# eBay/Sequence-Semantic-Embedding

Hardware: AMD Instinct MI355X
Metric: encoded seqs/sec (+ query x target cosine-scores/sec, top-1 vs ref) (higher is better)
Workload: dtype f32; 1 GPU; configs[1]: classification stand-in, dual-encoder LSTM H=S=256 E=50 T=32 V=32000; encode 16384 source seqs/GPU/step + cosine top-10 vs 571-target index; batch_per_gpu=16384, seq_len=32, targets=571, parallelism=dp1, weights=random-init (reference initialisers, seed 0)

## Files before the change

### sequence-semantic-embedding_amd/csrc/score_topk.hip

```cpp
#include <cstdlib>

#include "sse_kernels.h"
#include "score_exact.h"

#define SC_THREADS 512
#define SC_KC 16
#ifndef SC_PRIO_K
#define SC_PRIO_K 1
#define SC_PRIO_E 0
#endif

#ifdef SSE_SCORE_CLOCK
#include <cstdio>
__device__ long long g_score_clk[8 * 8];
#define SC_CLK_DECL long long ck_[8] = {0, 0, 0, 0, 0, 0, 0, 0}, ck_t = clock64();
#define SC_CLK(i)                   \
  {                                 \
    const long long n_ = clock64(); \
    ck_[i] += n_ - ck_t;            \
    ck_t = n_;                      \
  }
#else
#define SC_CLK_DECL
#define SC_CLK(i)
// ... 1093 lines not shown
bool score_small_index_applies(int Q, int KG, int64_t NT) {
  return Q >= 1024 && (KG == 32 || KG == 8 || KG == 7) && NT * 32 <= 1024 && (size_t)32 * (NT * 32 + 1) * sizeof(float) <= (size_t)144 * 1024;
}
hipError_t launch_score_small_index(const SmallIndexArgs &a, hipStream_t stream) {
  if (!score_small_index_applies(a.Q, a.KG, a.NT)) return hipErrorInvalidValue;
  const size_t lds = (size_t)32 * (a.NT * 32 + 1) * sizeof(float);
  const dim3 grid((a.Q + 31) / 32), block(256);
  auto go = [&](auto kernel) -> hipError_t {
    hipError_t e = hipFuncSetAttribute(reinterpret_cast<const void *>(kernel), hipFuncAttributeMaxDynamicSharedMemorySize, (int)lds);
    if (e != hipSuccess) return e;
    hipLaunchKernelGGL(kernel, grid, block, lds, stream, a);
    return hipGetLastError();
  };
  if (a.idx_x3 && a.KG != 32) return go(score_small_index_x3_kernel<4>);
  if (a.KG == 8) return go(score_small_index_kernel<8>);
  if (a.KG == 7) return go(score_small_index_kernel<7>);
  const hipError_t e32 = a.idx_x3 ? go(score_small_index_x3_kernel<16>) : go(score_small_index_kernel<32>);
  if (e32 != hipSuccess) return e32;
#ifdef SSE_SCORE_CLOCK
  if (a.Q >= 8192) {
    static int n = 0;
    if (n++ % 8 == 3) {
      long long v[64];
      (void)hipStreamSynchronize(stream);
      (void)hipMemcpyFromSymbol(v, HIP_SYMBOL(g_score_clk), sizeof v);
      for (int w = 0; w < 4; w += 3)
        fprintf(stderr, "[small index clock Q=%d NT=%d] wave %d cycles: query fragments %lld | scores (MFMA + LDS stores) %lld | barrier %lld | selection: loads + bounds %lld | bisection %lld | winners + rank + stores %lld (both batches)\n",
                a.Q, a.NT, w, v[w * 8 + 0], v[w * 8 + 1], v[w * 8 + 2], v[w * 8 + 5], v[w * 8 + 6], v[w * 8 + 3] + v[w * 8 + 4]);
    }
  }
#endif
  return hipGetLastError();
}

hipError_t launch_score_topk(const ScoreArgs &a_in, hipStream_t stream) {
  ScoreArgs a = a_in;
#ifdef SSE_SCORE_MEASURE
  {
    static const int dbg = getenv("SSE_SCORE_DBG") ? atoi(getenv("SSE_SCORE_DBG")) : 0;
    a.dbg = dbg;
  }
#endif
  if (a.KC != SC_KC) return hipErrorInvalidValue;
  if (a.q_rows && ((a.NQ != 1 && !a.COLLECT) || a.S < 1)) return hipErrorInvalidValue;
  if (a.NSPLIT > 8 && (a.NSPLIT & 7)) return hipErrorInvalidValue;
  if (a.NSPLIT < 8 && (8 % a.NSPLIT)) return hipErrorInvalidValue;
  if (a.COLLECT) {
    if (!a.lane_max && (!a.col_thr || !a.col_slot || !a.col_cnt || !a.col_buf)) return hipErrorInvalidValue;
    if (a.BF) return a.NQ == 4 ? launch_score_variant<4, true, true>(a, stream) : hipErrorInvalidValue;
    if (a.NQ == 1) return launch_score_variant<1, false, true>(a, stream);
    if (a.NQ == 2) return launch_score_variant<2, false, true>(a, stream);
    if (a.NQ == 4) return launch_score_variant<4, false, true>(a, stream);
    return hipErrorInvalidValue;
  }
  if (!a.part_bnd) return hipErrorInvalidValue;
  if (a.BF) {
    if (a.NQ == 1) return launch_score_variant<1, true, false>(a, stream);
    if (a.NQ == 2) return launch_score_variant<2, true, false>(a, stream);
    if (a.NQ == 4) return launch_score_variant<4, true, false>(a, stream);
    return hipErrorInvalidValue;
  }
  if (a.NQ == 1) return launch_score_variant<1, false, false>(a, stream);
  if (a.NQ == 2) return launch_score_variant<2, false, false>(a, stream);
  if (a.NQ == 4) return launch_score_variant<4, false, false>(a, stream);
  return hipErrorInvalidValue;
}


template <int NB>
__device__ __forceinline__ int packed_value_of_lane(int lane) {
  int v = 0;
#pragma unroll
  for (int cnt = NB, bit = 5; cnt > 1; cnt >>= 1, --bit) v = v * 2 + ((lane >> bit) & 1);
  return v;
}
template <int NB>
__device__ __forceinline__ int packed_lane_of_value(int v) {
  int lane = 0;
#pragma unroll
  for (int cnt = NB, bit = 5; cnt > 1; cnt >>= 1, --bit) lane |= ((v / (cnt / 2)) & 1) << bit;
  return lane;
}
template <int NB>
__device__ __forceinline__ double wave_exact_dot_packed(const float *qrow, const float *idxp, const double *idx64, const int64_t (&n)[NB],
                                                        int S, int KG, int lane, const float *idx_rm = nullptr) {
  static_assert(NB == 2 || NB == 4 || NB == 8, "power of two");
  double acc[NB];
#pragma unroll
  for (int b = 0; b < NB; ++b) acc[b] = 0.0;
  if (idx64) {
    for (int d = lane; d < S; d += 64) {
      double rv[NB];
#pragma unroll
      for (int b = 0; b < NB; ++b) rv[b] = idx64[(size_t)n[b] * S + d];
#pragma unroll
      for (int b = 0; b < NB; ++b) acc[b] += (double)qrow[d] * rv[b];
    }
  } else {
    for (int j = lane; j < KG * 2; j += 64) {
      const int kg = j >> 1, half = j & 1;
      f32x4 v[NB];
#pragma unroll
      for (int b = 0; b < NB; ++b)
        v[b] = idx_rm ? *reinterpret_cast<const f32x4 *>(idx_rm + (size_t)n[b] * S + j * 4)
                      : *reinterpret_cast<const f32x4 *>(idxp + (size_t)(n[b] >> 5) * KG * 256 + kg * 256 + (half * 32 + (int)(n[b] & 31)) * 4);
      const int d0 = kg * 8 + half * 4;
#pragma unroll
      for (int e = 0; e < 4; ++e)
        if (d0 + e < S) {
#pragma unroll
          for (int b = 0; b < NB; ++b) acc[b] += (double)qrow[d0 + e] * (double)v[b][e];
        }
    }
  }
  int m = 32;
#pragma unroll
  for (int cnt = NB; cnt > 1; cnt >>= 1, m >>= 1) {
    const bool up = (lane & m) != 0;
#pragma unroll
    for (int i = 0; i < cnt / 2; ++i) {
      const double send = up ? acc[i] : acc[i + cnt / 2];
      const double keep = up ? acc[i + cnt / 2] : acc[i];
      acc[i] = keep + __shfl_xor(send, m);
    }
  }
#pragma unroll
  for (; m > 0; m >>= 1) acc[0] += __shfl_xor(acc[0], m);
  return acc[0];
}

#define RS_THREADS 256
#define RS_MAXWIN 256
#define RS_MAXNC 4096
__global__ __launch_bounds__(RS_THREADS) void rescore_kernel(RescoreArgs a) {
  __shared__ int s_cnt;
  __shared__ int s_wid[RS_MAXWIN];
  __shared__ double s_ex[RS_MAXWIN];
  __shared__ float s_m[RS_THREADS / 64];
  __shared__ double s_qn[RS_THREADS / 64];
  extern __shared__ __attribute__((aligned(16))) unsigned long long s_key[];
  const int q = blockIdx.x, tid = threadIdx.x, lane = tid & 63, w = tid >> 6;
  if (a.uncert_clear && q == 0 && tid == 0) *a.uncert_clear = 0;
  if (a.q_count && q >= *a.q_count) return;
  const int qo = a.qmap ? a.qmap[q] : q;
  const float *ps = a.part_scores + (size_t)q * a.NC;
  const int32_t *pi = a.part_ids + (size_t)q * a.NC;
  const float *qrow = a.q + (size_t)q * a.S;
  const int KG = (a.S + 7) / 8;

  constexpr int PER = RS_MAXNC / RS_THREADS;
  float rs[PER];
  int ri[PER];
#pragma unroll
  for (int j = 0; j < PER; ++j) {
    const int c = tid + j * RS_THREADS;
    ri[j] = (c < a.NC) ? pi[c] : -1;
    rs[j] = (c < a.NC) ? ps[c] : NEG_INF;
  }
  float mmax = NEG_INF;
  for (int c = tid; c < a.NC / SC_KC; c += RS_THREADS) mmax = fmaxf(mmax, a.part_bnd[(size_t)q * (a.NC / SC_KC) + c]);

  {
    double v = 0.0;
    for (int d = tid; d < a.S; d += RS_THREADS) v += (double)qrow[d] * qrow[d];
#pragma unroll
    for (int o = 32; o > 0; o >>= 1) v += __shfl_xor(v, o);
    if (lane == 0) s_qn[w] = v;
  }
#pragma unroll
  for (int o = 32; o > 0; o >>= 1) mmax = fmaxf(mmax, __shfl_xor(mmax, o));
  if (lane == 0) s_m[w] = mmax;
  if (tid == 0) s_cnt = 0;

#pragma unroll
  for (int j = 0; j < PER; ++j) {
    const int c = tid + j * RS_THREADS;
    if (c < a.NC) {
      unsigned u = __float_as_uint(rs[j]);
      u = (u & 0x80000000u) ? ~u : (u | 0x80000000u);
      s_key[c] = (ri[j] < 0) ? 0ull : (((unsigned long long)u << 32) | (unsigned long long)(0xFFFFFFFFu - (unsigned)ri[j]));
    }
  }
  __syncthreads();
  const float qnorm = (float)sqrt(s_qn[0] + s_qn[1] + s_qn[2] + s_qn[3]);
  const float eps_q = a.eps * qnorm;
  mmax = fmaxf(fmaxf(s_m[0], s_m[1]), fmaxf(s_m[2], s_m[3]));
  float kth = NEG_INF;
  if (a.NC <= 256) {
    const unsigned long long key = (tid < a.NC) ? s_key[tid] : 0ull;
    int rank = 0;
    for (int j = 0; j < a.NC; ++j) rank += (s_key[j] > key) ? 1 : 0;
    float mine = (key != 0ull && rank == a.k - 1) ? rs[0] : NEG_INF;
#pragma unroll
    for (int o = 32; o > 0; o >>= 1) mine = fmaxf(mine, __shfl_xor(mine, o));
    __shared__ float s_thr[RS_THREADS / 64];
    if (lane == 0) s_thr[w] = mine;
    __syncthreads();
    kth = fmaxf(fmaxf(s_thr[0], s_thr[1]), fmaxf(s_thr[2], s_thr[3]));
  } else {
    __shared__ unsigned long long s_best[(RS_THREADS / 64) * SC_KC];
    const int nslots = a.NC / SC_KC;
    int head[RS_MAXNC / SC_KC / RS_THREADS];
#pragma unroll
    for (int j = 0; j < RS_MAXNC / SC_KC / RS_THREADS; ++j) head[j] = 0;
    for (int it = 0; it < a.k; ++it) {
      unsigned long long best = 0ull;
#pragma unroll
      for (int j = 0; j < RS_MAXNC / SC_KC / RS_THREADS; ++j) {
        const int slot = tid + j * RS_THREADS;
        if (slot < nslots && head[j] < SC_KC) {
          const unsigned long long key = s_key[slot * SC_KC + head[j]];
// ... 125 lines not shown
#endif
  const bool have = lane < a.NC;
  const int id = have ? a.part_ids[(size_t)q * a.NC + lane] : -1;
  const float sc = have ? a.part_scores[(size_t)q * a.NC + lane] : NEG_INF;
  const float bnd = (lane < a.NC / SC_KC) ? a.part_bnd[(size_t)q * (a.NC / SC_KC) + lane] : NEG_INF;
  double qn = 0.0;
  for (int d = lane; d < a.S; d += 64) qn += (double)qrow[d] * qrow[d];
#pragma unroll
  for (int o = 32; o > 0; o >>= 1) qn += __shfl_xor(qn, o);
  const float qnorm = (float)sqrt(qn);
  const float eps_q = a.eps * qnorm;
  RS_CLK(0)

  unsigned u = __float_as_uint(sc);
  u = (u & 0x80000000u) ? ~u : (u | 0x80000000u);
  const unsigned long long key = (id < 0) ? 0ull : (((unsigned long long)u << 32) | (unsigned long long)(0xFFFFFFFFu - (unsigned)id));
  const int key_lo = (int)(unsigned)key, key_hi = (int)(unsigned)(key >> 32);
  int rank = 0;
  for (int j = 0; j < a.NC; ++j) {
    const unsigned long long kj = ((unsigned long long)(unsigned)__builtin_amdgcn_readlane(key_hi, j) << 32) |
                                  (unsigned long long)(unsigned)__builtin_amdgcn_readlane(key_lo, j);
    rank += (kj > key) ? 1 : 0;
  }
  const unsigned long long kmask = __ballot(key != 0ull && rank == a.k - 1);
  const float kth = kmask ? __int_as_float(__builtin_amdgcn_readlane(__float_as_int(sc), __ffsll((long long)kmask) - 1)) : NEG_INF;
  const bool in_win = (id >= 0) && (sc >= kth - 2.0f * eps_q);
  float mmax = NEG_INF;
  for (int j = 0; j < a.NC / SC_KC; ++j) mmax = fmaxf(mmax, __int_as_float(__builtin_amdgcn_readlane(__float_as_int(bnd), j)));
  const unsigned long long wmask = __ballot(in_win);
  const int nwin = __popcll(wmask);
  const int mi = __popcll(wmask & ((1ull << lane) - 1ull));
  const int idm = __builtin_amdgcn_ds_permute((in_win ? mi : 63) * 4, id);
  RS_CLK(1)
  double exm = -__builtin_inf();
  for (int m0 = 0; m0 < nwin; m0 += RS_NB) {
    int64_t n[RS_NB];
#pragma unroll
    for (int c = 0; c < RS_NB; ++c) n[c] = __builtin_amdgcn_readlane(idm, (m0 + c < nwin) ? m0 + c : 0);
    const double tot = wave_exact_dot_packed<RS_NB>(qrow, a.idx32, a.idx64, n, a.S, KG, lane, a.idx_rm);
    const int want = lane - m0;
    const double got = __shfl(tot, packed_lane_of_value<RS_NB>(want & (RS_NB - 1)));
    if (want >= 0 && want < RS_NB && lane < nwin) exm = got;
  }
  RS_CLK(2)
  int r2 = 0;
  for (int j = 0; j < nwin; ++j)
    r2 += before(readlane_f64(exm, j), (int64_t)__builtin_amdgcn_readlane(idm, j), exm, (int64_t)idm) ? 1 : 0;
  const bool member = lane < nwin;
  if (member && r2 < a.k) {
    a.out_scores[(size_t)qo * a.k + r2] = exm;
    a.out_ids[(size_t)qo * a.k + r2] = a.id_base + idm;
    if (a.host_flag) {
      a.host_scores[(size_t)qo * a.k + r2] = exm;
      a.host_ids[(size_t)qo * a.k + r2] = a.id_base + idm;
    }
  }
  const unsigned long long tmask = __ballot(member && r2 == a.k - 1);
  const double theta = tmask ? readlane_f64(exm, __ffsll((long long)tmask) - 1) : -__builtin_inf();
  if (a.host_flag) __threadfence_system();
  RS_CLK(3)
#ifdef SSE_SCORE_CLOCK
  if (q == a.Q / 2 && lane == 0) {
    rk_[4] = nwin;
    for (int i = 0; i < 6; ++i) g_score_clk[i] = rk_[i];
  }
#endif
  if (lane == 0) {
    const bool ok = (nwin >= a.k) && ((double)mmax + (double)eps_q < theta);
    a.cert[qo] = ok ? 1 : 0;
    if (!ok && a.uncert) atomicAdd(a.uncert, 1);
    if (a.col_thr) a.col_thr[qo] = ok ? __builtin_inff() : __double2float_rd(theta - (double)(a.eps32 * qnorm));
    if (a.col_slot) {
      a.col_slot[qo] = ok ? -1 : qo;
      a.col_cnt[qo] = 0;
    }
    if (a.host_flag) {
      a.host_cert[qo] = ok ? 1 : 0;
      if (qo == 0 && a.host_err) *a.host_err = a.err_in ? *a.err_in : 0;
      __hip_atomic_store(a.host_flag + qo, a.seq, __ATOMIC_RELEASE, __HIP_MEMORY_SCOPE_SYSTEM);
    }
  }
}

hipError_t launch_rescore(const RescoreArgs &a, hipStream_t stream) {
  if (a.NC > RS_MAXNC) return hipErrorInvalidValue;
  if (a.NC <= 64) {
    hipLaunchKernelGGL(rescore_small_kernel, dim3((a.Q + 3) / 4), dim3(256), 0, stream, a);
#ifdef SSE_SCORE_CLOCK
    if (a.Q >= 8192) {
      static int n = 0;
      if (n++ % 8 == 3) {
        long long v[8];
        (void)hipStreamSynchronize(stream);
        (void)hipMemcpyFromSymbol(v, HIP_SYMBOL(g_score_clk), sizeof v);
        fprintf(stderr, "[rescore_small clock Q=%d NC=%d] cycles: query norm %lld | candidates, rank, k-th, window %lld | float64 dots %lld (window of %lld) | exact rank + outputs %lld\n",
                a.Q, a.NC, v[0], v[1], v[2], v[4], v[3]);
      }
    }
#endif
    return hipGetLastError();
  }
  hipLaunchKernelGGL(rescore_kernel, dim3(a.Q), dim3(RS_THREADS), (size_t)a.NC * sizeof(unsigned long long), stream, a);
  return hipGetLastError();
}

#define EX_THREADS 256
struct ExactArgs {
  const float *q;
  const float *idxp;
  const double *idx64;
  const int32_t *cert;
  double *out_scores;
  int64_t *out_ids;
  int64_t id_base, N;
  int32_t Q, S, k;
  int32_t k_off, k_total;
  unsigned long long *served;
  const int32_t *uncert;
};

__device__ __forceinline__ void exact_topk_query(const ExactArgs a, const int q, double (*s_sc)[SC_KC],
                                                 int64_t (*s_id)[SC_KC]) {
  const int tid = threadIdx.x, lane = tid & 63, w = tid >> 6;
  if (a.served && tid == 0 && a.k_off == 0) atomicAdd(a.served, 1ull);
  const float *qrow = a.q + (size_t)q * a.S;
  const int KG = (a.S + 7) / 8;
  double ls[SC_KC];
  int64_t li[SC_KC];
#pragma unroll
  for (int i = 0; i < SC_KC; ++i) {
    ls[i] = -__builtin_inf();
    li[i] = -1;
  }
  double cut_s = __builtin_inf();
  int64_t cut_id = -1;
  if (a.k_off > 0) {
    cut_s = a.out_scores[(size_t)q * a.k_total + a.k_off - 1];
    cut_id = a.out_ids[(size_t)q * a.k_total + a.k_off - 1] - a.id_base;
  }
  for (int64_t n = w; n < a.N; n += EX_THREADS / 64) {
    double s = wave_exact_dot(qrow, a.idxp, a.idx64, n, a.S, KG, lane);
    const bool after_cut = (s < cut_s) || (s == cut_s && n > cut_id);
    if (after_cut && s > ls[SC_KC - 1]) {
      int64_t id = n;
      bool ins = false;
#pragma unroll
      for (int i = 0; i < SC_KC; ++i) {
        const bool gt = ins || (s > ls[i]);
        ins = gt;
        const double tv = ls[i];
        const int64_t ti = li[i];
        ls[i] = gt ? s : tv;
        li[i] = gt ? id : ti;
        s = gt ? tv : s;
        id = gt ? ti : id;
      }
    }
  }
  if (lane == 0) {
#pragma unroll
    for (int i = 0; i < SC_KC; ++i) {
      s_sc[w][i] = ls[i];
      s_id[w][i] = li[i];
    }
  }
  __syncthreads();
  if (tid == 0) {
    unsigned pos4 = 0;
// ... 285 lines not shown
```

### sequence-semantic-embedding_amd/csrc/sse_api.hip

```cpp
#include <cmath>
#include <cstdarg>
#include <cstdio>
#include <cstdlib>
#include <algorithm>
#include <chrono>
#include <cstring>
#include <dlfcn.h>
#include <link.h>
#include <mutex>
#include <string>
#include <vector>

#include "../../include/sse_hip.h"
#include "sse_kernels.h"
#include "train.h"

namespace {

thread_local std::string g_create_error;

struct Variable {
  std::string name;
  int rows = 0, cols = 0;
  int64_t count = 0;
// ... 36 lines not shown
  size_t cap = 0;
  DevBuf() = default;
  DevBuf(const DevBuf &) = delete;
  DevBuf &operator=(const DevBuf &) = delete;
  ~DevBuf() {
    if (p) (void)hipFree(p);
  }
};

struct TrainState {
  DevBuf ids[2], labels, raw[2], draw[2], tape_g[2], tape_a[2], h_last[2], dh_last[2], dg_a[2], dg_b[2], db_part[2],
      dk_part[2], dm_part[2], sq_part, norm_part, row_loss, row_acc, scal;
  DevBuf feat_rm, pos, dfeat, dw_part, dbias_part, wt, wct;
  uint64_t gen_ver[2] = {0, 0};
  DevBuf gen_A[2], gen_tape[2], gen_dG[2], gen_hl[2], gen_KT[2], gen_Kq[2], gen_MT[2], gen_G, gen_c, gen_dA, gen_dc, gen_dkp;
  hipStream_t side[2] = {nullptr, nullptr};
  hipEvent_t ev_fork = nullptr, ev_join[2] = {nullptr, nullptr};
  float *KhT[2] = {nullptr, nullptr}, *KxT[2] = {nullptr, nullptr};
  unsigned short *KhT16[2] = {nullptr, nullptr};
  unsigned short *KxT16[2] = {nullptr, nullptr};
  bool packed_dirty = true;
  bool fp32_dirty = true;
  float *arena = nullptr;
  bool arena_external = false, grads_ready = false;
  DevBuf corpus[2], rows[2];
  int64_t corpus_N[2] = {0, 0};
  int32_t corpus_T[2] = {0, 0};
  bool rows_mode = false;
  bool defer_err = false;
  DevBuf ids_raw[2], perm, hot_part[2];
  int perm_B = 0;
  std::vector<int32_t> h_perm, h_rows[2], h_tgt;
  std::vector<float> h_labels;
};

}

enum { PATH_PERSIST, PATH_CLUSTER, PATH_SMALL, PATH_X3, PATH_GENERIC, PATH_FWD, PATH_FWD_ROWS32, PATH_FWD_ROWS64, PATH_FWD_GS, PATH_FWD_XT,
       PATH_COUNT };

struct sse_handle {
  sse_config cfg;
  std::mutex mu;
  std::string err;
  std::vector<Variable> vars;
  Encoder enc[2];
  bool packed_dirty = true;
  uint64_t weights_version = 1;
  bool mp_fresh = false;
  int pad_skip = 1;
  int pad_sort_dev = 1;
  int score_two_pass_min_rows = 49152, score_two_pass_rows = 524288;
  int64_t two_pass_calls = 0;
  DevBuf s_lmax;
  int lstm_gate_split = 1;
  DevBuf s_padzero, s_padwork, s_padorder;
  int32_t *pad_stat = nullptr;
  int32_t pad_seq = 0;
  int64_t pad_sorted_calls = 0;
  int64_t lstm_path_calls[PATH_COUNT] = {};
  int lstm_x3 = 0;
  unsigned short *emb16 = nullptr;
  bool emb16_valid = false;
  int lstm_persist_rows = 32;
  uint32_t persist_epoch = 0;
  hipStream_t stream = nullptr;
  int persist_inject = 0;
  int64_t persist_fallbacks = 0;
  int cu_count = 0;
  int lstm_cluster_rows = 1024;
  uint32_t cluster_epoch = 0;
  int lstm_cluster_chunks = 3;
  int cluster_backoff = -1;
  int cluster_skip[2] = {0, 0};
  int lstm_cluster_coop = 1;
  int lstm_cluster_wt = 0;
  int lstm_cluster_drop = 0;
  int lstm_small_rows = 1024;
  int lstm_x_table = 1;
  int lstm_x_table_mb = 256;
  int64_t x_table_builds = 0;
  int score_small_index = 1;
  int score_small_x3 = 1;
  int score_bf16 = 1;
  void *idxp16 = nullptr;
  size_t idxp16_cap = 0;
  bool idxp16_valid = false;
  bool fb_cnt_init = false;
  int uncert_word = 0;
  bool cnn_bf16 = false;
  unsigned short *emb_bf16 = nullptr, *cnn_Wc16 = nullptr, *cnn_Mx3 = nullptr;
  int lstm_train_rows = 0;
  int train_bwd_x3 = 0;
  int train_fwd_x3 = 0;
  int train_dk_x3 = 0;
  int train_generic = 0;
  int train_gen1 = 0;
  int train_pair_dedup = 1;
  int train_serial = 0;
  float *emb_pad = nullptr;
  int cnn_W[4] = {-1, -1, -1, -1}, cnn_b[4] = {-1, -1, -1, -1}, cnn_M = -1, tgt_table = -1;
  float *cnn_Wc = nullptr, *cnn_bias = nullptr, *cnn_Mp = nullptr;
  int32_t *err_flag = nullptr;
  float *idxp = nullptr;
  size_t idxp_cap = 0;
  double *idx64 = nullptr;
  DevBuf idx_rm;
  bool idx_rm_valid = false;
  DevBuf idx_x3;
  bool idx_x3_valid = false;
  int64_t idx_N = 0, idx_base = 0;
  int idx_S = 0;
  float idx_norm_max = 1.0f;
  DevBuf s_ids, s_out, s_q, s_qp, s_ps, s_pi, s_cert, s_os, s_oi, s_tmp, s_tmp2, s_feat, s_zero, s_map;
  DevBuf s_qmap, s_qc;
  DevBuf s_qp32, s_fb_cnt;
  DevBuf g_A, g_G, g_c, g_hl, g_raw;
  DevBuf g_KT[2], g_Kq[2], g_MT[2];
  uint64_t g_ver[2] = {0, 0};
  DevBuf s_xchg;
  DevBuf s_persist;
  DevBuf s_cluster;
  int32_t *pin_small = nullptr;
  void *pin = nullptr;
  size_t pin_cap = 0;
  int32_t score_seq = 0;
  DevBuf s_pb, s_cthr, s_cslot, s_ccnt, s_cbuf;
  DevBuf s_rk, s_rk_cnt;
  bool rk_cnt_init = false;
  DevBuf s_ab, s_ab_sort, s_ab_cnt, s_ab_out;
  bool ab_cnt_init = false;
  DevBuf idx_tags, idx_tag_sum, s_ft_max, s_ft_cnt;
  bool tags_set = false, ft_cnt_init = false;
  int score_filtered_skip = 1;
  DevBuf idx_groups, s_gp_max, s_gp_cnt;
  bool groups_set = false, gp_cnt_init = false;
  DevBuf s_af_bnd, s_af_cnt;
  bool af_cnt_init = false;
  DevBuf s_stage;
  int eval_chunk_rows = 65536;
  int64_t eval_paired_calls = 0;
  DevBuf ev_ids[2], ev_stage, ev_rows[2], ev_labels, ev_raw[2], ev_row, ev_sums;
  float lr = 0.9f;
  int64_t global_step = 0;
  TrainState *train = nullptr;
  std::vector<hipEvent_t> events;
};

namespace {

int fail(sse_handle *h, const char *fmt, ...) {
  char buf[512];
  va_list ap;
  va_start(ap, fmt);
  vsnprintf(buf, sizeof buf, fmt, ap);
  va_end(ap);
  if (h) h->err = buf; else g_create_error = buf;
  return 1;
}

#define HIPCHECK(h, expr)                                                                         \
  do {                                                                                            \
    hipError_t e_ = (expr);                                                                       \
    if (e_ != hipSuccess) return fail(h, "%s failed: %s (%s:%d)", #expr, hipGetErrorString(e_), __FILE__, __LINE__); \
  } while (0)

// ... 1345 lines not shown
    HIPCHECK(h, launch_exact_topk(q, h->idxp, h->idx64, (const int32_t *)h->s_cert.p, out_s, out_i, h->idx_base, h->idx_N, Q, S, k, st,
                                  counters + 2));
    if (split) *split = 0;
    return 0;
  }
  const int POOL = std::min(Q, 1024);
  if (reserve(h, h->s_qp, (size_t)QB * NQ * KG * 256 * sizeof(float))) return 1;
  if (reserve(h, h->s_ps, (size_t)Q * (bf ? NCmax : NC) * sizeof(float))) return 1;
  if (reserve(h, h->s_pi, (size_t)Q * (bf ? NCmax : NC) * sizeof(int32_t))) return 1;
  if (reserve(h, h->s_pb, (size_t)Q * (bf ? NCmax / 16 : nsplit) * sizeof(float))) return 1;
  if (reserve(h, h->s_cert, (size_t)Q * sizeof(int32_t))) return 1;
  if (reserve_collect(h, Q, POOL)) return 1;
  if (split) *split = 1;
  const bool first = phase != SCORE_REST, rest = phase != SCORE_FIRST;
  const bool rows_direct = NQ == 1;
  if (first && !rows_direct && !small_idx) {
    if (bf) HIPCHECK(h, launch_pack_rows_bf16(q, Q, S, h->s_qp.p, st));
    else HIPCHECK(h, launch_pack_rows(q, Q, S, (float *)h->s_qp.p, st));
  }
  ScoreArgs a;
  if (rows_direct) {
    a.q_rows = q;
    a.S = S;
  }
  a.BF = bf ? 1 : 0;
  a.idxp = bf ? (const float *)h->idxp16 : h->idxp;
  a.qp = (const float *)h->s_qp.p;
  a.part_scores = (float *)h->s_ps.p;
  a.part_ids = (int32_t *)h->s_pi.p;
  a.part_bnd = (float *)h->s_pb.p;
  a.N = h->idx_N;
  a.Q = Q;
  a.KG = bf ? KG16 : KG;
  a.NT = (int)NT;
  a.QT = QT;
  a.NSPLIT = nsplit;
  a.KC = 16;
  a.NQ = NQ;
  if (first) {
    if (small_idx) {
      SmallIndexArgs si{q, h->idxp, a.part_scores, a.part_ids, a.part_bnd, h->idx_N, Q, S, KG, (int)NT};
      if (small_x3) si.idx_x3 = h->idx_x3.p;
      HIPCHECK(h, launch_score_small_index(si, st));
    } else {
      HIPCHECK(h, launch_score_topk(a, st));
    }
  }
  RescoreArgs r;
  r.q = q;
  r.idx32 = h->idxp;
  r.idx64 = h->idx64;
  r.idx_rm = h->idx_rm_valid ? (const float *)h->idx_rm.p : nullptr;
  r.part_scores = a.part_scores;
  r.part_ids = a.part_ids;
  r.part_bnd = a.part_bnd;
  r.out_scores = out_s;
  r.out_ids = out_i;
  r.cert = (int32_t *)h->s_cert.p;
  r.id_base = h->idx_base;
  r.N = h->idx_N;
  r.Q = Q;
  r.S = S;
  r.NC = NC;
  r.k = k;
  const float eps32 = score_eps32(h);
  r.eps = eps32;
  r.eps32 = eps32;
  r.col_thr = (float *)h->s_cthr.p;
  if (first) h->uncert_word ^= 1;
  int32_t *const uncert = (int32_t *)(counters + 4) + h->uncert_word;
  const int follow_grid = 2 * (h->cu_count > 0 ? h->cu_count : 256);
  r.uncert = uncert;
  r.uncert_clear = (int32_t *)(counters + 4) + (h->uncert_word ^ 1);
  const bool own_slots = Q <= POOL;
  if (own_slots) {
    r.col_slot = (int32_t *)h->s_cslot.p;
    r.col_cnt = (int32_t *)h->s_ccnt.p;
  }
  if (bf) r.eps += (float)(1.02 * (1.0 / 256.0 + 1.0 / 262144.0) * h->idx_norm_max);
  if (small_x3)
    r.eps = (float)(((1.0 + 1.0 / 64.0) / 32768.0 + 2.0 * (3 * S + 2) * 5.97e-8 * (1.0 + 1.0 / 32.0)) * h->idx_norm_max);
  if (first) {
    RescoreArgs rf = r;
    if (mirror) {
      rf.host_scores = mirror->scores;
      rf.host_ids = mirror->ids;
      rf.host_cert = mirror->cert;
      rf.host_err = mirror->err;
      rf.host_flag = mirror->flag;
      rf.err_in = h->err_flag;
      rf.seq = mirror->seq;
    }
    HIPCHECK(h, launch_rescore(rf, st));
  }
  if (!rest) return 0;
  const float *qp32 = (const float *)h->s_qp.p;
  if (bf && Q > 32) {
    if (reserve(h, h->s_qp32, (size_t)QB * NQ * KG * 256 * sizeof(float))) return 1;
    if (reserve(h, h->s_qmap, (size_t)(Q + 1) * sizeof(int32_t))) return 1;
    if (reserve(h, h->s_qc, (size_t)QT * 32 * S * sizeof(float))) return 1;
    HIPCHECK(h, launch_count_uncert(r.cert, Q, counters, st));
    int32_t *qmap = (int32_t *)h->s_qmap.p, *qcount = qmap + Q;
    HIPCHECK(h, launch_compact_uncert(q, r.cert, Q, S, qmap, qcount, (float *)h->s_qc.p, st));
    if (!rows_direct) HIPCHECK(h, launch_pack_rows((const float *)h->s_qc.p, Q, S, (float *)h->s_qp32.p, st));
    ScoreArgs a2 = a;
    a2.BF = 0;
    a2.idxp = h->idxp;
    a2.qp = (const float *)h->s_qp32.p;
    if (rows_direct) a2.q_rows = (const float *)h->s_qc.p;
    a2.KG = KG;
    a2.q_count = qcount;
    a2.NSPLIT = nsplit2;
    HIPCHECK(h, launch_score_topk(a2, st));
    RescoreArgs r2 = r;
    r2.q = (const float *)h->s_qc.p;
    r2.NC = nsplit2 * 16;
    r2.eps = eps32;
    r2.qmap = qmap;
    r2.q_count = qcount;
    r2.uncert = r2.uncert_clear = nullptr;
    HIPCHECK(h, launch_rescore(r2, st));
    qp32 = (const float *)h->s_qp32.p;
  }
  if (!own_slots) {
    HIPCHECK(h, hipMemsetAsync(h->s_ccnt.p, 0, (size_t)(POOL + 1) * sizeof(int32_t), st));
    HIPCHECK(h, launch_assign_slots(r.cert, Q, POOL, (int32_t *)h->s_cslot.p, (int32_t *)h->s_ccnt.p + POOL, st));
  }
  ScoreArgs c = a;
  c.BF = 0;
  c.idxp = h->idxp;
  c.qp = qp32;
  c.q_rows = q;
  c.S = S;
  c.KG = KG;
  c.COLLECT = 1;
  c.col_thr = (const float *)h->s_cthr.p;
  c.col_slot = (const int32_t *)h->s_cslot.p;
  c.col_cnt = (int32_t *)h->s_ccnt.p;
  c.col_buf = (int32_t *)h->s_cbuf.p;
  c.col_cap = SSE_COLLECT_CAP;
  c.uncert = uncert;
  HIPCHECK(h, launch_score_topk(c, st));
  SelectArgs sel{q, h->idxp, h->idx64, c.col_slot, c.col_cnt, c.col_buf, SSE_COLLECT_CAP, out_s, out_i, r.cert, h->idx_base, Q, S, k,
                 counters + 1, uncert, follow_grid};
  HIPCHECK(h, launch_select_topk(sel, st));
  HIPCHECK(h, launch_exact_topk(q, h->idxp, h->idx64, r.cert, out_s, out_i, h->idx_base, h->idx_N, Q, S, k, st, counters + 2, uncert,
                                follow_grid));
  return 0;
}

}

extern "C" {

const char *sse_last_error(sse_handle *h) { return h ? h->err.c_str() : g_create_error.c_str(); }

int sse_create(const sse_config *cfg, sse_handle **out) {
  if (!cfg || !out) return fail(nullptr, "sse_create: null argument");
  *out = nullptr;
  int ndev = 0;
  if (hipGetDeviceCount(&ndev) != hipSuccess || ndev == 0) return fail(nullptr, "no HIP device available");
  if (cfg->device < 0 || cfg->device >= ndev) return fail(nullptr, "device %d out of range (have %d)", cfg->device, ndev);
  if (cfg->vocab_size < 2 || cfg->embedding_size < 1 || cfg->encoding_size < 1)
    return fail(nullptr, "bad model sizes V=%d E=%d S=%d", cfg->vocab_size, cfg->embedding_size, cfg->encoding_size);
  sse_handle *h = new sse_handle();
  h->cfg = *cfg;
// ... 349 lines not shown
  if (bits) {
    if (check_err_flag(h, nullptr, &bits)) return 1;
    if (bits == 4) {
      if (encode_fallback_locked(h, side, B, T, normalize, nullptr)) return 1;
      if (score_to_host_locked(h, (const float *)h->s_out.p, B, k, out_scores, out_ids)) return 1;
    }
  }
  if (enc_out_host)
    HIPCHECK(h, hipMemcpy(enc_out_host, h->s_out.p, (size_t)B * h->cfg.encoding_size * sizeof(float), hipMemcpyDeviceToHost));
  return 0;
}

namespace {

struct DevCounters {
  DevBuf sse_handle::*buf;
  bool sse_handle::*init;
  int words;
};
enum { CG_RANK, CG_ABOVE, CG_FILTERED, CG_GROUPED, CG_AFTER, CG_TOPK, CG_DEV_COUNT, CG_HOST = CG_DEV_COUNT, CG_PATH, CG_COOP };
const DevCounters DEV_COUNTERS[CG_DEV_COUNT] = {
    {&sse_handle::s_rk_cnt, &sse_handle::rk_cnt_init, 2}, {&sse_handle::s_ab_cnt, &sse_handle::ab_cnt_init, 3},
    {&sse_handle::s_ft_cnt, &sse_handle::ft_cnt_init, 3}, {&sse_handle::s_gp_cnt, &sse_handle::gp_cnt_init, 3},
    {&sse_handle::s_af_cnt, &sse_handle::af_cnt_init, 3}, {&sse_handle::s_fb_cnt, &sse_handle::fb_cnt_init, 4}};
int64_t sse_handle::*const HOST_COUNTERS[] = {&sse_handle::persist_fallbacks, &sse_handle::two_pass_calls, &sse_handle::pad_sorted_calls,
                                              &sse_handle::eval_paired_calls, &sse_handle::x_table_builds};

const struct {
  const char *name;
  int group, word;
} COUNTERS[] = {
    {"lstm_persist_fallbacks", CG_HOST, 0},
    {"score_two_pass_calls", CG_HOST, 1},
    {"pad_sorted_calls", CG_HOST, 2},
    {"eval_paired_calls", CG_HOST, 3},
    {"lstm_x_table_builds", CG_HOST, 4},
    {"lstm_path_persist", CG_PATH, PATH_PERSIST},
    {"lstm_path_cluster", CG_PATH, PATH_CLUSTER},
    {"lstm_path_small", CG_PATH, PATH_SMALL},
    {"lstm_path_x3", CG_PATH, PATH_X3},
    {"lstm_path_generic", CG_PATH, PATH_GENERIC},
    {"lstm_path_fwd", CG_PATH, PATH_FWD},
    {"lstm_fwd_rows32", CG_PATH, PATH_FWD_ROWS32},
    {"lstm_fwd_rows64", CG_PATH, PATH_FWD_ROWS64},
    {"lstm_fwd_gate_split", CG_PATH, PATH_FWD_GS},
    {"lstm_fwd_x_table", CG_PATH, PATH_FWD_XT},
    {"lstm_coop_refused", CG_COOP, 0},
    {"score_rank_band_rows", CG_RANK, 0},
    {"score_rank_bruteforce_pairs", CG_RANK, 1},
    {"score_above_band_rows", CG_ABOVE, 0},
    {"score_above_bruteforce_pairs", CG_ABOVE, 1},
    {"score_above_long_segments", CG_ABOVE, 2},
    {"score_filtered_collected_rows", CG_FILTERED, 0},
    {"score_filtered_bruteforce_queries", CG_FILTERED, 1},
    {"score_filtered_tiles_skipped", CG_FILTERED, 2},
    {"score_grouped_collected_rows", CG_GROUPED, 0},
    {"score_grouped_bruteforce_queries", CG_GROUPED, 1},
    {"score_after_collected_rows", CG_AFTER, 0},
    {"score_after_bruteforce_queries", CG_AFTER, 1},
    {"score_bf16_second_chance_queries", CG_TOPK, 0},
    {"score_collect_queries", CG_TOPK, 1},
    {"score_bruteforce_queries", CG_TOPK, 2},
};

static int read_dev_counter(sse_handle *h, const DevCounters &g, int word, int64_t *value) {
  unsigned long long v[4] = {0, 0, 0, 0};
  if ((h->*g.buf).p && h->*g.init) {
    HIPCHECK(h, hipSetDevice(h->cfg.device));
    HIPCHECK(h, hipDeviceSynchronize());
    HIPCHECK(h, hipMemcpy(v, (h->*g.buf).p, g.words * sizeof v[0], hipMemcpyDeviceToHost));
  }
  *value = (int64_t)v[word];
  return 0;
}

const struct {
  const char *name;
  int sse_handle::*member;
  int min, max;
  const char *message;
} OPTIONS[] = {
    {"score_small_index", &sse_handle::score_small_index},
    {"score_small_x3", &sse_handle::score_small_x3},
    {"score_filtered_skip", &sse_handle::score_filtered_skip},
    {"score_bf16", &sse_handle::score_bf16},
    {"train_bwd_x3", &sse_handle::train_bwd_x3},
    {"train_fwd_x3", &sse_handle::train_fwd_x3},
    {"train_dk_x3", &sse_handle::train_dk_x3},
    {"train_generic", &sse_handle::train_generic},
    {"train_gen1", &sse_handle::train_gen1},
    {"train_pair_dedup", &sse_handle::train_pair_dedup},
    {"train_serial", &sse_handle::train_serial},
    {"pad_skip", &sse_handle::pad_skip},
    {"lstm_gate_split", &sse_handle::lstm_gate_split},
    {"lstm_x3", &sse_handle::lstm_x3},
    {"lstm_persist_inject_miss", &sse_handle::persist_inject},
    {"lstm_cluster_drop_wg", &sse_handle::lstm_cluster_drop},
    {"lstm_cluster_coop", &sse_handle::lstm_cluster_coop},
    {"lstm_cluster_write_through", &sse_handle::lstm_cluster_wt},
    {"score_two_pass_min_rows", &sse_handle::score_two_pass_min_rows, 0, INT32_MAX, "score_two_pass_min_rows must be >= 0"},
    {"score_two_pass_rows", &sse_handle::score_two_pass_rows, 0, INT32_MAX, "score_two_pass_rows must be >= 0"},
    {"pad_sort_dev", &sse_handle::pad_sort_dev, 0, 2, "pad_sort_dev must be 0 (off), 1 (adaptive) or 2 (always)"},
    {"lstm_persist_rows", &sse_handle::lstm_persist_rows, 0, INT32_MAX, "lstm_persist_rows must be >= 0"},
    {"lstm_cluster_chunks", &sse_handle::lstm_cluster_chunks, 1, INT32_MAX, "lstm_cluster_chunks must be >= 1"},
    {"lstm_cluster_rows", &sse_handle::lstm_cluster_rows, 0, INT32_MAX, "lstm_cluster_rows must be >= 0"},
    {"lstm_small_rows", &sse_handle::lstm_small_rows, 0, INT32_MAX, "lstm_small_rows must be >= 0"},
    {"lstm_x_table", &sse_handle::lstm_x_table, 0, 2, "lstm_x_table must be 0 (off), 1 (batches with B * T >= vocab_size) or 2 (always)"},
    {"lstm_x_table_mb", &sse_handle::lstm_x_table_mb, 0, INT32_MAX, "lstm_x_table_mb must be >= 0"},
};

}

int sse_get_counter(sse_handle *h, const char *name, int64_t *value) {
  if (!h || !name || !value) return 1;
  std::lock_guard<std::mutex> lk(h->mu);
  for (const auto &c : COUNTERS) {
    if (strcmp(name, c.name) != 0) continue;
    if (c.group < CG_DEV_COUNT) return read_dev_counter(h, DEV_COUNTERS[c.group], c.word, value);
    *value = c.group == CG_HOST ? h->*HOST_COUNTERS[c.word] : c.group == CG_PATH ? h->lstm_path_calls[c.word] : (int64_t)lstm_coop_refused();
    return 0;
  }
  return fail(h, "unknown counter '%s'", name);
}

int sse_set_option(sse_handle *h, const char *name, int32_t value) {
  if (!h || !name) return 1;
  std::lock_guard<std::mutex> lk(h->mu);
  for (const auto &o : OPTIONS) {
    if (strcmp(name, o.name) != 0) continue;
    if (o.message && (value < o.min || value > o.max)) return fail(h, "%s", o.message);
    h->*o.member = o.message ? value : value != 0;
    return 0;
  }
  if (strcmp(name, "cnn_bf16") == 0) {
    if (h->cfg.network_mode != SSE_MODE_SOURCE_ONLY_CNN) return fail(h, "option cnn_bf16 needs network_mode source_only_cnn");
    h->cnn_bf16 = value != 0;
    h->packed_dirty = true;
    h->mp_fresh = false;
    return 0;
  }
  if (strcmp(name, "lstm_train_rows") == 0) {
    if (value != 0 && value != 32 && value != 64) return fail(h, "lstm_train_rows must be 0, 32 or 64");
    h->lstm_train_rows = (int)value;
    return 0;
  }
  if (strcmp(name, "eval_chunk_rows") == 0) {
    if (value < 2) return fail(h, "eval_chunk_rows must be >= 2");
    h->eval_chunk_rows = (int)(value & ~1);
    return 0;
  }
  if (strcmp(name, "lstm_persist_epoch") == 0) {
    if (value < 0 || value >= (1 << 20)) return fail(h, "lstm_persist_epoch must be in [0, 2^20)");
    h->persist_epoch = (uint32_t)value;
    return 0;
  }
  if (strcmp(name, "lstm_cluster_backoff") == 0) {
    if (value < -1) return fail(h, "lstm_cluster_backoff must be >= 0 (or -1: automatic)");
    h->cluster_backoff = (int)value;
    h->cluster_skip[0] = h->cluster_skip[1] = 0;
    return 0;
  }
  return fail(h, "unknown option '%s'", name);
}

int sse_l2_normalize_dev(sse_handle *h, const float *x_dev, float *out_dev, int64_t rows, int32_t cols, void *stream) {
  SSE_ENTER(h);
// ... 1279 lines not shown
```

### sequence-semantic-embedding_amd/csrc/sse_kernels.h

```cpp
#pragma once
#include <hip/hip_runtime.h>
#include <stdint.h>

typedef float f32x4 __attribute__((ext_vector_type(4)));
typedef float f32x16 __attribute__((ext_vector_type(16)));

__host__ __device__ static inline int frag32_off(int r_in_tile, int k_in_group) {
  return ((((k_in_group >> 2) << 5) + r_in_tile) << 2) + (k_in_group & 3);
}

__device__ static inline int mfma_row(int reg, int lane) { return (reg & 3) + 8 * (reg >> 2) + 4 * (lane >> 5); }

static inline int round_up(int x, int m) { return (x + m - 1) / m * m; }

typedef unsigned int sse_u32x4 __attribute__((ext_vector_type(4)));
__host__ __device__ static inline unsigned short sse_bf16_rne(float f) {
  unsigned u;
  __builtin_memcpy(&u, &f, 4);
  u += 0x7FFFu + ((u >> 16) & 1u);
  return (unsigned short)(u >> 16);
}
__host__ __device__ static inline float sse_bf16_f32(unsigned short h) {
  const unsigned u = (unsigned)h << 16;
  float f;
// ... 175 lines not shown
  int32_t B, T, V, E, Ep, KGx, KGh, H, Hp, S, NTS, normalize;
  const float *pad_h = nullptr, *pad_c = nullptr;
  int32_t pad_stride = 0;
  unsigned long long *hx = nullptr;
  unsigned long long *sx = nullptr;
  uint32_t epoch = 0;
  int32_t NCL = 0;
  int32_t write_through = 0;
  int32_t plain_launch = 0;
  int32_t drop_wg = 0;
};
int lstm_cluster_ok(int E, int H, int S);
int lstm_cluster_max_rows();
size_t lstm_cluster_weight_floats(int E, int H);
size_t lstm_cluster_hx_words(int H);
size_t lstm_cluster_sx_words();
hipError_t launch_pack_lstm_cluster(const float *K, const float *b, int E, int H, float *Wc, hipStream_t stream);
hipError_t launch_lstm_cluster(const LstmClusterArgs &a, hipStream_t stream);

struct ScoreArgs {
  const float *idxp;
  const float *qp;
  float *part_scores;
  int32_t *part_ids;
  float *part_bnd;
  int64_t N;
  int32_t Q, KG, NT, QT, NSPLIT, KC;
  int32_t NQ = 4;
  int32_t thr_off = 0;
  const int32_t *q_count = nullptr;
  int32_t BF = 0;
  int32_t COLLECT = 0;
  const float *col_thr = nullptr;
  const int32_t *col_slot = nullptr;
  int32_t *col_cnt = nullptr;
  int32_t *col_buf = nullptr;
  int32_t col_cap = 0;
  float *lane_max = nullptr;
  int32_t dbg = 0;
  const float *q_rows = nullptr;
  int32_t S = 0;
  const int32_t *uncert = nullptr;
};
hipError_t launch_score_topk(const ScoreArgs &a, hipStream_t stream);
hipError_t launch_lane_max_threshold(const float *q, const float *lane_max, int Q, int S, int NV, float eps, float *col_thr,
                                     int32_t *col_slot, hipStream_t st);
#define SSE_MAX_INDEX_DIM 1024
int score_pick_nq(int Q, int S, int with_bf16);
size_t score_lds_bytes(int NQ, int KG, int BF, int COLLECT);
hipError_t launch_pack_rows_bf16(const float *rows, int64_t R, int C, void *out, hipStream_t stream);
hipError_t launch_count_uncert(const int32_t *cert, int Q, unsigned long long *count, hipStream_t st);
hipError_t launch_compact_uncert(const float *q, const int32_t *cert, int Q, int S, int32_t *qmap, int32_t *count, float *qc,
                                 hipStream_t st);
hipError_t launch_frag32_to_bf16(const float *idxp, int64_t NT, int KG, void *out, hipStream_t stream);
hipError_t launch_frag32_to_split_bf16(const float *idxp, int64_t NT, int KG, void *out, hipStream_t stream);

#define SSE_COLLECT_CAP 4096
#define SSE_MAX_SELECT_K 1024

struct RescoreArgs {
  const float *q;
  const float *idx32;
  const double *idx64;
  const float *part_scores;
  const int32_t *part_ids;
  const float *part_bnd;
  double *out_scores;
  int64_t *out_ids;
  int32_t *cert;
  int64_t id_base, N;
  int32_t Q, S, NC, k;
  float eps;
  const int32_t *qmap = nullptr, *q_count = nullptr;
  float *col_thr = nullptr;
  float eps32 = 0.0f;
  int32_t *col_slot = nullptr, *col_cnt = nullptr;
  double *host_scores = nullptr;
  int64_t *host_ids = nullptr;
  int32_t *host_cert = nullptr, *host_flag = nullptr, *host_err = nullptr;
  const int32_t *err_in = nullptr;
  int32_t seq = 0;
  const float *idx_rm = nullptr;
  int32_t *uncert = nullptr, *uncert_clear = nullptr;
};
hipError_t launch_rescore(const RescoreArgs &a, hipStream_t stream);

struct SmallIndexArgs {
  const float *q_rows;
  const float *idxp;
  float *part_scores;
  int32_t *part_ids;
  float *part_bnd;
  int64_t N;
  int32_t Q, S, KG, NT;
  const void *idx_x3 = nullptr;
};
bool score_small_index_applies(int Q, int KG, int64_t NT);
hipError_t launch_score_small_index(const SmallIndexArgs &a, hipStream_t stream);

struct RankArgs {
  const float *q;
  const int32_t *pair_q;
  const int64_t *pair_id;
  const double *pair_score_in;
  const float *idxp;
  const double *idx64;
  int64_t *out_before;
  double *out_score;
  double *thr64;
  float *lo, *hi;
  unsigned long long *sure;
  int32_t *band_cnt, *band_buf;
  int32_t band_cap;
  const int32_t *bad;
  unsigned long long *counters;
  int64_t id_base, N;
  int32_t S, KG, NT, P, NSPLIT, NQ;
  float eps32;
};
hipError_t launch_rank_validate(const int32_t *pair_q, const int64_t *pair_id, int64_t L, int Q, int need_row, int64_t id_base,
                                int64_t N, int32_t *bad, int32_t *err_flag, hipStream_t st);
hipError_t launch_score_rank(const RankArgs &a, hipStream_t st);

struct AboveArgs {
  const float *q;
  const int32_t *pair_q;
  const double *pair_thr;
  const float *idxp;
  const double *idx64;
  float *lo, *hi;
  unsigned long long *sure;
  int32_t *band_cnt, *band_buf;
  int32_t band_cap;
  const int32_t *bad;
  int32_t *err_flag;
  unsigned long long *counters;
  int64_t *counts;
  const int64_t *offsets;
  const int64_t *total;
  int32_t *ovf;
  unsigned long long *cursor;
  int64_t *out_ids;
  int64_t cap;
  int64_t id_base, N;
  int32_t S, KG, NT, P, NSPLIT, NQ, emit;
  float eps32;
};
#define SSE_ABOVE_SORT_CAP 8192
hipError_t launch_above_validate(const int32_t *pair_q, int64_t L, int Q, int32_t *bad, int32_t *err_flag, hipStream_t st);
hipError_t launch_score_above(const AboveArgs &a, hipStream_t st);
hipError_t launch_above_scan(int64_t *offsets, int64_t L, const int32_t *bad, hipStream_t st);
struct AboveListArgs {
  const float *q;
  const int32_t *pair_q;
  const float *idxp;
  const double *idx64;
  const int64_t *offsets;
  const unsigned long long *cursor;
  int64_t *ids;
  double *scores;
  int64_t *scratch_ids;
  double *scratch_scores;
  const int32_t *bad;
  int32_t *err_flag;
  unsigned long long *counters;
  int64_t L, cap, id_base, N;
// ... 129 lines not shown
```

Before: 7.578 million seqs/s.

## Add row-packed rescore kernel handling four queries per wavefront with DPP ranking

Adds a specialised rescore kernel for 16-candidate partial results. Each 16-lane row of a wavefront handles one query, so four queries share a wave. Candidates are ranked with DPP row rotations instead of shared-memory sorting, and ranking is skipped when the small-index path already sorted them. Exact float64 dots are batched across the combined windows of all four queries, with double-buffered row loads. It is gated on NC==16, no qmap or host mirroring, and Q>=256, with an option flag to turn it off. The aim is to cut per-query block overhead and idle lanes, at the cost of extra code complexity.

```diff
diff --git a/sequence-semantic-embedding_amd/csrc/score_topk.hip b/sequence-semantic-embedding_amd/csrc/score_topk.hip
--- a/sequence-semantic-embedding_amd/csrc/score_topk.hip
+++ b/sequence-semantic-embedding_amd/csrc/score_topk.hip
@@ -1199,6 +1199,23 @@
   return lane;
 }
 template <int NB>
+__device__ __forceinline__ double packed_reduce(double (&acc)[NB], int lane) {
+  int m = 32;
+#pragma unroll
+  for (int cnt = NB; cnt > 1; cnt >>= 1, m >>= 1) {
+    const bool up = (lane & m) != 0;
+#pragma unroll
+    for (int i = 0; i < cnt / 2; ++i) {
+      const double send = up ? acc[i] : acc[i + cnt / 2];
+      const double keep = up ? acc[i + cnt / 2] : acc[i];
+      acc[i] = keep + __shfl_xor(send, m);
+    }
+  }
+#pragma unroll
+  for (; m > 0; m >>= 1) acc[0] += __shfl_xor(acc[0], m);
+  return acc[0];
+}
+template <int NB>
 __device__ __forceinline__ double wave_exact_dot_packed(const float *qrow, const float *idxp, const double *idx64, const int64_t (&n)[NB],
                                                         int S, int KG, int lane, const float *idx_rm = nullptr) {
   static_assert(NB == 2 || NB == 4 || NB == 8, "power of two");
@@ -1230,20 +1247,52 @@
         }
     }
   }
-  int m = 32;
-#pragma unroll
-  for (int cnt = NB; cnt > 1; cnt >>= 1, m >>= 1) {
-    const bool up = (lane & m) != 0;
-#pragma unroll
-    for (int i = 0; i < cnt / 2; ++i) {
-      const double send = up ? acc[i] : acc[i + cnt / 2];
-      const double keep = up ? acc[i + cnt / 2] : acc[i];
-      acc[i] = keep + __shfl_xor(send, m);
-    }
-  }
-#pragma unroll
-  for (; m > 0; m >>= 1) acc[0] += __shfl_xor(acc[0], m);
-  return acc[0];
+  return packed_reduce<NB>(acc, lane);
+}
+template <int NB>
+__device__ __forceinline__ double wave_exact_dot_packed_rows(const float *const (&qr)[NB], const float *idxp, const double *idx64,
+                                                             const int64_t (&n)[NB], int S, int KG, int lane, const float *idx_rm, bool vec) {
+  static_assert(NB == 2 || NB == 4 || NB == 8, "power of two");
+  double acc[NB];
+#pragma unroll
+  for (int b = 0; b < NB; ++b) acc[b] = 0.0;
+  if (idx64) {
+    for (int d = lane; d < S; d += 64) {
+      double rv[NB];
+      float qv[NB];
+#pragma unroll
+      for (int b = 0; b < NB; ++b) {
+        rv[b] = idx64[(size_t)n[b] * S + d];
+        qv[b] = qr[b][d];
+      }
+#pragma unroll
+      for (int b = 0; b < NB; ++b) acc[b] += (double)qv[b] * rv[b];
+    }
+  } else {
+    for (int j = lane; j < KG * 2; j += 64) {
+      const int kg = j >> 1, half = j & 1;
+      const int d0 = kg * 8 + half * 4;
+      f32x4 v[NB], qv[NB];
+#pragma unroll
+      for (int b = 0; b < NB; ++b) {
+        v[b] = idx_rm ? *reinterpret_cast<const f32x4 *>(idx_rm + (size_t)n[b] * S + j * 4)
+                      : *reinterpret_cast<const f32x4 *>(idxp + (size_t)(n[b] >> 5) * KG * 256 + kg * 256 + (half * 32 + (int)(n[b] & 31)) * 4);
+        if (vec) {
+          qv[b] = (d0 < S) ? *reinterpret_cast<const f32x4 *>(qr[b] + d0) : f32x4{0, 0, 0, 0};
+        } else {
+#pragma unroll
+          for (int e = 0; e < 4; ++e) qv[b][e] = (d0 + e < S) ? qr[b][d0 + e] : 0.0f;
+        }
+      }
+#pragma unroll
+      for (int e = 0; e < 4; ++e)
+        if (d0 + e < S) {
+#pragma unroll
+          for (int b = 0; b < NB; ++b) acc[b] += (double)qv[b][e] * (double)v[b][e];
+        }
+    }
+  }
+  return packed_reduce<NB>(acc, lane);
 }
 
 #define RS_THREADS 256
@@ -1535,8 +1584,162 @@
   }
 }
 
+template <int R>
+__device__ __forceinline__ int row_ror(int v) {
+  return __builtin_amdgcn_update_dpp(v, v, 0x120 + R, 0xF, 0xF, false);
+}
+#define RS_ROW_ROTATIONS(X) X(1) X(2) X(3) X(4) X(5) X(6) X(7) X(8) X(9) X(10) X(11) X(12) X(13) X(14) X(15)
+__global__ __launch_bounds__(256) void rescore_rows_kernel(RescoreArgs a) {
+  __shared__ f32x4 rs_qf[4][4][64];
+  const int lane = threadIdx.x & 63, g = lane >> 4, c = lane & 15;
+  const int q0 = (blockIdx.x * 4 + (threadIdx.x >> 6)) * 4;
+  if (a.uncert_clear && blockIdx.x == 0 && threadIdx.x == 0) *a.uncert_clear = 0;
+  if (q0 >= a.Q) return;
+  const int q = q0 + g;
+  const bool live = q < a.Q;
+  const int KG = (a.S + 7) / 8;
+  const float *qbase = a.q + (size_t)q0 * a.S;
+  const int id = live ? a.part_ids[(size_t)q0 * 16 + lane] : -1;
+  const float sc = live ? a.part_scores[(size_t)q0 * 16 + lane] : NEG_INF;
+  const float bnd = (live && c == 0) ? a.part_bnd[q] : NEG_INF;
+  double qn4[4] = {0.0, 0.0, 0.0, 0.0};
+  for (int d = lane; d < a.S; d += 64) {
+    float x[4];
+#pragma unroll
+    for (int j = 0; j < 4; ++j) x[j] = qbase[(size_t)(q0 + j < a.Q ? j : 0) * a.S + d];
+#pragma unroll
+    for (int j = 0; j < 4; ++j) qn4[j] += (double)x[j] * x[j];
+  }
+#pragma unroll
+  for (int o = 32; o > 0; o >>= 1) {
+#pragma unroll
+    for (int j = 0; j < 4; ++j) qn4[j] += __shfl_xor(qn4[j], o);
+  }
+  const double qn = g == 0 ? qn4[0] : g == 1 ? qn4[1] : g == 2 ? qn4[2] : qn4[3];
+  const float qnorm = (float)sqrt(qn);
+  const float eps_q = a.eps * qnorm;
+
+  const bool valid = id >= 0;
+  int rank = c;
+  if (!a.sorted) {
+    unsigned u = __float_as_uint(sc);
+    u = (u & 0x80000000u) ? ~u : (u | 0x80000000u);
+    const unsigned long long key = valid ? (((unsigned long long)u << 32) | (unsigned long long)(0xFFFFFFFFu - (unsigned)id)) : 0ull;
+    const int key_lo = (int)(unsigned)key, key_hi = (int)(unsigned)(key >> 32);
+    rank = 0;
+#define RS_RANK_STEP(R)                                                                                      \
+  {                                                                                                          \
+    const unsigned long long kj = ((unsigned long long)(unsigned)row_ror<R>(key_hi) << 32) |                 \
+                                  (unsigned long long)(unsigned)row_ror<R>(key_lo);                          \
+    rank += (kj > key) ? 1 : 0;                                                                              \
+  }
+    RS_ROW_ROTATIONS(RS_RANK_STEP)
+#undef RS_RANK_STEP
+  }
+  const int sh = g * 16, row0 = lane & 48;
+  const unsigned kf = (unsigned)(__ballot(valid && rank == a.k - 1) >> sh) & 0xFFFFu;
+  const float kth_s = __shfl(sc, row0 + (kf ? __ffs((int)kf) - 1 : 0));
+  const float kth = kf ? kth_s : NEG_INF;
+  const bool in_win = valid && (sc >= kth - 2.0f * eps_q);
+  const float mmax = fmaxf(NEG_INF, bnd);
+  const unsigned long long wmask = __ballot(in_win);
+  const int nw = __popcll(wmask);
+  const int nwin = __popc((unsigned)(wmask >> sh) & 0xFFFFu);
+  const int mi = __popcll(wmask & ((1ull << lane) - 1ull));
+  const int idm = __builtin_amdgcn_ds_permute((in_win ? mi : 63) * 4, id);
+  const int gm = __builtin_amdgcn_ds_permute((in_win ? mi : 63) * 4, g);
+  const bool vec = (a.S & 3) == 0 && (reinterpret_cast<uintptr_t>(a.q) & 15) == 0;
+  double exm = -__builtin_inf();
+  if (vec && !a.idx64 && KG * 2 <= 64) {
+    const bool act = lane < KG * 2 && lane * 4 < a.S;
+    const int d0 = act ? lane * 4 : 0;
+    f32x4(*qf)[64] = rs_qf[threadIdx.x >> 6];
+#pragma unroll
+    for (int j = 0; j < 4; ++j) qf[j][lane] = *reinterpret_cast<const f32x4 *>(qbase + (size_t)(q0 + j < a.Q ? j : 0) * a.S + d0);
+    const bool rm = a.idx_rm != nullptr;
+    const float *rows = (rm ? a.idx_rm : a.idx32) + (rm ? d0 : (act ? (lane >> 1) * 256 + (lane & 1) * 128 : 0));
+    const size_t tile = (size_t)KG * 256;
+    auto row_of = [&](int m) -> f32x4 {
+      const int n = __builtin_amdgcn_readlane(idm, m);
+      return *reinterpret_cast<const f32x4 *>(rows + (rm ? (size_t)n * a.S : (size_t)(n >> 5) * tile + (size_t)((n & 31) * 4)));
+    };
+    auto batch = [&](int m0, const f32x4(&cur)[RS_NB], f32x4(&nxt)[RS_NB]) {
+#pragma unroll
+      for (int b = 0; b < RS_NB; ++b) nxt[b] = row_of(m0 + RS_NB + b < nw ? m0 + RS_NB + b : 0);
+      double acc[RS_NB];
+#pragma unroll
+      for (int b = 0; b < RS_NB; ++b) {
+        const f32x4 qv = qf[__builtin_amdgcn_readlane(gm, (m0 + b < nw) ? m0 + b : 0)][lane];
+        double s = 0.0;
+#pragma unroll
+        for (int e = 0; e < 4; ++e) s += (double)qv[e] * (double)cur[b][e];
+        acc[b] = act ? s : 0.0;
+      }
+      const double tot = packed_reduce<RS_NB>(acc, lane);
+      const int want = mi - m0;
+      const double got = __shfl(tot, packed_lane_of_value<RS_NB>(want & (RS_NB - 1)));
+      if (in_win && want >= 0 && want < RS_NB) exm = got;
+    };
+    f32x4 va[RS_NB], vb[RS_NB];
+#pragma unroll
+    for (int b = 0; b < RS_NB; ++b) va[b] = row_of(b < nw ? b : 0);
+    for (int m0 = 0; m0 < nw; m0 += 2 * RS_NB) {
+      batch(m0, va, vb);
+      if (m0 + RS_NB < nw) batch(m0 + RS_NB, vb, va);
+    }
+  } else {
+    for (int m0 = 0; m0 < nw; m0 += RS_NB) {
+      int64_t n[RS_NB];
+      const float *qr[RS_NB];
+#pragma unroll
+      for (int b = 0; b < RS_NB; ++b) {
+        const int m = (m0 + b < nw) ? m0 + b : 0;
+        n[b] = __builtin_amdgcn_readlane(idm, m);
+        qr[b] = qbase + (size_t)__builtin_amdgcn_readlane(gm, m) * a.S;
+      }
+      const double tot = wave_exact_dot_packed_rows<RS_NB>(qr, a.idx32, a.idx64, n, a.S, KG, lane, a.idx_rm, vec);
+      const int want = mi - m0;
+      const double got = __shfl(tot, packed_lane_of_value<RS_NB>(want & (RS_NB - 1)));
+      if (in_win && want >= 0 && want < RS_NB) exm = got;
+    }
+  }
+  const long long exb = __double_as_longlong(exm);
+  const int ex_lo = (int)exb, ex_hi = (int)(exb >> 32), idw = in_win ? id : -1;
+  int r2 = 0;
+#define RS_EXACT_STEP(R)                                                                                     \
+  {                                                                                                          \
+    const int oi = row_ror<R>(idw);                                                                          \
+    const double oe = __longlong_as_double(((long long)row_ror<R>(ex_hi) << 32) | (unsigned int)row_ror<R>(ex_lo)); \
+    r2 += (oi >= 0 && before(oe, (int64_t)oi, exm, (int64_t)id)) ? 1 : 0;                                    \
+  }
+  RS_ROW_ROTATIONS(RS_EXACT_STEP)
+#undef RS_EXACT_STEP
+  if (in_win && r2 < a.k) {
+    a.out_scores[(size_t)q * a.k + r2] = exm;
+    a.out_ids[(size_t)q * a.k + r2] = a.id_base + id;
+  }
+  const unsigned tf = (unsigned)(__ballot(in_win && r2 == a.k - 1) >> sh) & 0xFFFFu;
+  const double theta_s = __shfl(exm, row0 + (tf ? __ffs((int)tf) - 1 : 0));
+  const double theta = tf ? theta_s : -__builtin_inf();
+  if (live && c == 0) {
+    const bool ok = (nwin >= a.k) && ((double)mmax + (double)eps_q < theta);
+    a.cert[q] = ok ? 1 : 0;
+    if (!ok && a.uncert) atomicAdd(a.uncert, 1);
+    if (a.col_thr) a.col_thr[q] = ok ? __builtin_inff() : __double2float_rd(theta - (double)(a.eps32 * qnorm));
+    if (a.col_slot) {
+      a.col_slot[q] = ok ? -1 : q;
+      a.col_cnt[q] = 0;
+    }
+  }
+}
+#undef RS_ROW_ROTATIONS
+
 hipError_t launch_rescore(const RescoreArgs &a, hipStream_t stream) {
   if (a.NC > RS_MAXNC) return hipErrorInvalidValue;
+  if (a.rows && a.NC == 16 && !a.qmap && !a.q_count && !a.host_flag && a.Q >= 256) {
+    hipLaunchKernelGGL(rescore_rows_kernel, dim3((a.Q + 15) / 16), dim3(256), 0, stream, a);
+    return hipGetLastError();
+  }
   if (a.NC <= 64) {
     hipLaunchKernelGGL(rescore_small_kernel, dim3((a.Q + 3) / 4), dim3(256), 0, stream, a);
 #ifdef SSE_SCORE_CLOCK
diff --git a/sequence-semantic-embedding_amd/csrc/sse_api.hip b/sequence-semantic-embedding_amd/csrc/sse_api.hip
--- a/sequence-semantic-embedding_amd/csrc/sse_api.hip
+++ b/sequence-semantic-embedding_amd/csrc/sse_api.hip
@@ -142,6 +142,7 @@
   int64_t x_table_builds = 0;
   int score_small_index = 1;
   int score_small_x3 = 1;
+  int score_rescore_rows = 1;
   int score_bf16 = 1;
   void *idxp16 = nullptr;
   size_t idxp16_cap = 0;
@@ -1653,6 +1654,8 @@
     r.eps = (float)(((1.0 + 1.0 / 64.0) / 32768.0 + 2.0 * (3 * S + 2) * 5.97e-8 * (1.0 + 1.0 / 32.0)) * h->idx_norm_max);
   if (first) {
     RescoreArgs rf = r;
+    rf.rows = h->score_rescore_rows != 0;
+    rf.sorted = small_idx;
     if (mirror) {
       rf.host_scores = mirror->scores;
       rf.host_ids = mirror->ids;
@@ -2168,6 +2171,7 @@
 } OPTIONS[] = {
     {"score_small_index", &sse_handle::score_small_index},
     {"score_small_x3", &sse_handle::score_small_x3},
+    {"score_rescore_rows", &sse_handle::score_rescore_rows},
     {"score_filtered_skip", &sse_handle::score_filtered_skip},
     {"score_bf16", &sse_handle::score_bf16},
     {"train_bwd_x3", &sse_handle::train_bwd_x3},
diff --git a/sequence-semantic-embedding_amd/csrc/sse_kernels.h b/sequence-semantic-embedding_amd/csrc/sse_kernels.h
--- a/sequence-semantic-embedding_amd/csrc/sse_kernels.h
+++ b/sequence-semantic-embedding_amd/csrc/sse_kernels.h
@@ -281,6 +281,7 @@
   int32_t seq = 0;
   const float *idx_rm = nullptr;
   int32_t *uncert = nullptr, *uncert_clear = nullptr;
+  bool rows = false, sorted = false;
 };
 hipError_t launch_rescore(const RescoreArgs &a, hipStream_t stream);
 
```

Result: no change. 7.641 million seqs/s (median of 6 runs) (+0.8%).
